# fxxJuses/MICFormer

Hardware: AMD Instinct MI355X
Metric: train volumes/sec (128^3 CT+MRI pair) (higher is better)
Workload: dtype bf16; 1 GPU; MicFormer base Head(embed_dim=48, depths 2-2-6-2, heads 3-6-12-24, window 2^3, 8 classes) full train step (fwd + MDiceLoss + bwd + Adam/cosine) on 128^3 CT+MR pairs, DropPath on; local_batch=2, global_batch=2, parallelism=dp1, launch=hipGraph replay (one graph)

## Files before the change

### micformer_amd/csrc/common.h

```cpp
#pragma once
#include <hip/hip_runtime.h>
#include <stdint.h>

#include "../../include/micformer_hip.h"
#include "gemm_core.h"

#define MICF_RETURN_LAUNCH()                          \
  do {                                                \
    return hipGetLastError() == hipSuccess ? MICF_OK : MICF_ELAUNCH; \
  } while (0)

namespace micf {

struct Options {
  int block_wave = 1;
  int block_recompute_h = 0;
  int block_debug = 0;
  int sample_tile = 1;
  int sample_e = -1;
  int cell_cap = -1;
  int tile_cap_hits = -1, tile_cap_cell = -1, tile_cap_voxel = -1;
};
Options& options();

struct Geo {
  int B, D, H, W;
  FastDiv fW, fH, fD;
  Geo() {}
  Geo(int B_, int D_, int H_, int W_) : B(B_), D(D_), H(H_), W(W_), fW((uint32_t)W_), fH((uint32_t)H_), fD((uint32_t)D_) {}
  __host__ __device__ int64_t tokens() const { return (int64_t)B * D * H * W; }
  __device__ __forceinline__ void decode(int t, int& b, int& d, int& h, int& w) const {
    uint32_t q, r;
    fW.divmod((uint32_t)t, q, r); w = (int)r;
    fH.divmod(q, q, r); h = (int)r;
    fD.divmod(q, q, r); d = (int)r; b = (int)q;
  }
  __device__ __forceinline__ int token(int b, int d, int h, int w) const { return ((b * D + d) * H + h) * W + w; }
};

__device__ __forceinline__ float wave_sum(float v) {
#pragma unroll
  for (int o = 32; o > 0; o >>= 1) v += __shfl_xor(v, o, 64);
  return v;
}

int colsum_atomic(const float* dy, const float* scale, int64_t rps, float* out, int64_t M, int N, hipStream_t s);

constexpr int kOffsetHidden = 16;
struct CellLists {
  int* count;
  int* ovf_count;
  int* list;
  int* ovf;
  int cap;
  float* w8;
};
struct SampleFwdSet { const float *h, *ln_g, *ln_b, *w1, *xa; float *flow, *xs; };
struct SampleBwdSet {
  const float *dxs, *h, *ln_g, *ln_b, *w1, *xa, *flow;
  float *dxa, *dh, *dln_g, *dln_b, *dw1;
  CellLists cl;
  float* partials;
};
int offset_sample_fwd_groups(const SampleFwdSet* sets, int n, int B, int D, int H, int W, int C, float eps, hipStream_t stream);
int offset_sample_bwd_groups(SampleBwdSet* sets, int n, int B, int D, int H, int W, int C, float eps, float* workspace,
                             int64_t workspace_floats, hipStream_t s, int phase = 0);
struct SampleFinishCall { const SampleBwdSet* sets; int n, B, D, H, W, C; float* workspace; int64_t workspace_floats; };
int offset_sample_finish_many(const SampleFinishCall* calls, int ncalls, hipStream_t s);

struct Conv3FwdSet { const float* x1; const float* x2; const float* w; const float* bias; float* y; float* wt; };
struct Conv3BwdSet { const float* dy; const float* w; float* wt; float* dx1; float* dx2; };
int conv3_fwd_x_groups(const Conv3FwdSet* sets, int n, int c1, int c2, int B, int D, int H, int W, int N, hipStream_t stream, int dtype,
                       int prepared, int y_zeroed);
bool conv3_fwd_x_splits(int B, int D, int H, int W, int c1, int c2);
int conv3_bwd_data_x_groups(const Conv3BwdSet* sets, int ng, int c1, int acc1, int c2, int acc2, int B, int D, int H, int W, int N,
                            hipStream_t stream, int dtype, int prepared);

int conv3_bwd_data_x(const float* dy, const float* w, float* wt, float* dx1, int c1, int acc1, float* dx2, int c2, int acc2, int B,
                     int D, int H, int W, int N, hipStream_t stream, int dtype = 0, int prepared = 0);

int64_t conv3_fwdx_workspace(int N, int c1, int c2);
int conv3_fwd_x(const float* x1, int c1, const float* x2, int c2, const float* w, const float* bias, float* y, float* wt, int B, int D,
                int H, int W, int N, hipStream_t stream, int dtype = 0, int prepared = 0);
int64_t conv3_wgradx_workspace(int B, int D, int H, int W, int N, int c1, int c2, int items = 1);
int conv3_wgradx_items(const float* const* dy, const float* const* x1, const float* const* x2, float* const* dw, float* const* dbias,
                       int n, int c1, int c2, int B, int D, int H, int W, int N, float* ws, int64_t ws_floats, hipStream_t stream,
                       int dtype);
int conv3_wgradx(const float* dy, const float* x1, int c1, const float* x2, int c2, float* dw, float* dbias, int B, int D, int H,
                 int W, int N, float* ws, int64_t ws_floats, hipStream_t stream, int dtype = 0);

}
```

### micformer_amd/csrc/linear_grouped.hip

```cpp
#include "common.h"
#include "gemm_dma.h"

namespace micf {

constexpr int kGroupMax = 32;
constexpr int kGroupChunk = 1024;

struct GItem {
  const float* a; const float* dy; const float* scale; float* out; float* dbias; float* dw;
  int M, N, K, rps;
  int tiles_i, tiles, splits, direct;
  int ldw, pad_;
  int64_t split_stride;
};
struct GArgs {
  int n;
  int end[kGroupMax];
  GItem it[kGroupMax];
};

template <bool BF16>
__global__ void __launch_bounds__(256) wgrad_grouped_kernel(const GArgs g) {
  __shared__ __attribute__((aligned(1024))) float Ps[kDmaNS * 64 * kDmaBR];
  __shared__ __attribute__((aligned(1024))) float Qs[kDmaNS * 64 * kDmaBR];
  const int total = g.end[g.n - 1];
  const int w = xcd_order(blockIdx.x, total);
  if (w >= total) return;
  int k = 0;
  while (k < g.n - 1 && w >= g.end[k]) ++k;
  const GItem& it = g.it[k];
  const int local = w - (k ? g.end[k - 1] : 0);
  const int split = local / it.tiles, t = local % it.tiles;
  const int bi = t % it.tiles_i, bj = t / it.tiles_i;
  const int i0 = bi * 64, j0 = bj * 64;
  const int tid = threadIdx.x, lane = tid & 63, wave = __builtin_amdgcn_readfirstlane(tid >> 6);
  const int li = lane & 15, lr = lane >> 4;
  const int r_begin = split * kGroupChunk;
  const int r_end = (r_begin + kGroupChunk < it.M) ? r_begin + kGroupChunk : it.M;
  const DmaOperand P{it.a, it.K, it.K}, Q{it.dy, it.N, it.N};
  const bool do_cs = (it.dbias != nullptr) && (bi == 0) && (tid < 64);

  f32x4 tot[4];
#pragma unroll
  for (int q = 0; q < 4; ++q) tot[q] = f32x4{0.f, 0.f, 0.f, 0.f};
  float ctot = 0.f;
  for (int r = r_begin; r < r_end;) {
    int seg_end = r_end;
    float s = 1.f;
    if (it.scale) {
      const int b = r / it.rps;
      s = it.scale[b];
      const int lim = (b + 1) * it.rps;
      if (lim < seg_end) seg_end = lim;
    }
    f32x4 acc[4];
#pragma unroll
    for (int q = 0; q < 4; ++q) acc[q] = f32x4{0.f, 0.f, 0.f, 0.f};
    float csum = 0.f;
    if (r != r_begin) __syncthreads();
    const int nslab = (seg_end - r) / kDmaBR;
    dma_tile_loop<true, true, kDmaNS, BF16>(P, Q, i0, j0, r, nslab, Ps, Qs, acc, do_cs, csum);
    for (int rr = r + nslab * kDmaBR; rr < seg_end; ++rr) {
      const int jq = j0 + 4 * li + wave;
      float dyv = jq < it.N ? it.dy[(int64_t)rr * it.N + jq] : 0.f;
      if constexpr (BF16) dyv = __uint_as_float(pack_bf16(dyv, 0.f) << 16);
#pragma unroll
      for (int v = 0; v < 4; ++v) {
        const int i = i0 + 16 * lr + 4 * v;
        if (i >= it.K) continue;
        float4 a4 = *reinterpret_cast<const float4*>(it.a + (int64_t)rr * it.K + i);
        if constexpr (BF16) {
          const unsigned lo = pack_bf16(a4.x, a4.y), hi = pack_bf16(a4.z, a4.w);
          a4 = make_float4(__uint_as_float(lo << 16), __uint_as_float(lo & 0xFFFF0000u), __uint_as_float(hi << 16), __uint_as_float(hi & 0xFFFF0000u));
        }
        acc[0][v] += dyv * a4.x; acc[1][v] += dyv * a4.y; acc[2][v] += dyv * a4.z; acc[3][v] += dyv * a4.w;
      }
      if (do_cs && j0 + tid < it.N) csum += it.dy[(int64_t)rr * it.N + j0 + tid];
    }
#pragma unroll
    for (int q = 0; q < 4; ++q) { tot[q][0] += s * acc[q][0]; tot[q][1] += s * acc[q][1]; tot[q][2] += s * acc[q][2]; tot[q][3] += s * acc[q][3]; }
    ctot += s * csum;
    r = seg_end;
  }
  if (do_cs && j0 + tid < it.N) atomicAdd(it.dbias + j0 + tid, ctot);
  const int j = j0 + 4 * li + wave;
  if (j >= it.N) return;
  float* base = it.direct ? it.dw : it.out + (int64_t)split * it.split_stride;
  const int ld = it.direct ? it.ldw : it.K;
#pragma unroll
  for (int v = 0; v < 4; ++v) {
    const int i = i0 + 16 * lr + 4 * v;
    if (i >= it.K) continue;
    float* p = base + (int64_t)j * ld + i;
    float4 o = make_float4(tot[0][v], tot[1][v], tot[2][v], tot[3][v]);
    if (i + 4 <= it.K) {
      if (it.direct) { const float4 old = *reinterpret_cast<const float4*>(p); o.x += old.x; o.y += old.y; o.z += old.z; o.w += old.w; }
      *reinterpret_cast<float4*>(p) = o;
    } else {
      const float e[4] = {o.x, o.y, o.z, o.w};
      for (int q = 0; q < it.K - i; ++q) p[q] = it.direct ? p[q] + e[q] : e[q];
    }
  }
}


constexpr int kB16Piece = 1024 + 64;
constexpr int kB16Stage = 4 * kB16Piece;
typedef short s16x4 __attribute__((ext_vector_type(4)));

__device__ __forceinline__ bf16x8 tr_frag(unsigned stage_piece, int li, int unit0) {
  const int r = li >> 2, u = unit0 + ((li & 3) >> 1);
  const unsigned a0 = stage_piece + (unsigned)((r * 8 + (u ^ (2 * ((r >> 1) & 1)))) * 16 + (li & 1) * 8);
  const unsigned a1 = a0 + 4 * 8 * 16;
  const s16x4 lo = __builtin_amdgcn_ds_read_tr16_b64_v4i16((__attribute__((address_space(3))) s16x4*)(uintptr_t)a0);
  const s16x4 hi = __builtin_amdgcn_ds_read_tr16_b64_v4i16((__attribute__((address_space(3))) s16x4*)(uintptr_t)a1);
  return bf16x8{lo[0], lo[1], lo[2], lo[3], hi[0], hi[1], hi[2], hi[3]};
}

__device__ __forceinline__ void dma16_b16(const uint16_t* gsrc, unsigned lds_byte) {
  dma16(reinterpret_cast<const float*>(gsrc), lds_byte);
}

__global__ void __launch_bounds__(256) wgrad_grouped_b16_kernel(const GArgs g) {
  __shared__ __attribute__((aligned(1024))) char Ps[kDmaNS * kB16Stage];
  __shared__ __attribute__((aligned(1024))) char Qs[kDmaNS * kB16Stage];
  const int total = g.end[g.n - 1];
  const int w = xcd_order(blockIdx.x, total);
  if (w >= total) return;
  int k = 0;
  while (k < g.n - 1 && w >= g.end[k]) ++k;
  const GItem& it = g.it[k];
  const int local = w - (k ? g.end[k - 1] : 0);
  const int split = local / it.tiles, t = local % it.tiles;
  const int bi = t % it.tiles_i, bj = t / it.tiles_i;
  const int i0 = bi * 64, j0 = bj * 64;
  const int tid = threadIdx.x, lane = tid & 63, wave = __builtin_amdgcn_readfirstlane(tid >> 6);
  const int li = lane & 15, lr = lane >> 4;
  const int r_begin = split * kGroupChunk;
  const int r_end = (r_begin + kGroupChunk < it.M) ? r_begin + kGroupChunk : it.M;
  const uint16_t* A = reinterpret_cast<const uint16_t*>(it.a);
  const uint16_t* DY = reinterpret_cast<const uint16_t*>(it.dy);
  const bool do_cs = (it.dbias != nullptr) && (bi == 0);

  const int srow = lane >> 3, sunit = (lane & 7) ^ (2 * ((srow >> 1) & 1));
  int xa = i0 + 8 * sunit; if (xa > it.K - 8) xa = it.K - 8;
  int xd = j0 + 8 * sunit; if (xd > it.N - 8) xd = it.N - 8;
  const unsigned pl = lds_addr(Ps) + wave * kB16Piece, ql = lds_addr(Qs) + wave * kB16Piece;
  const unsigned pf = lds_addr(Ps) + lr * kB16Piece, qf = lds_addr(Qs) + lr * kB16Piece;

  f32x4 tot[4];
#pragma unroll
  for (int q = 0; q < 4; ++q) tot[q] = f32x4{0.f, 0.f, 0.f, 0.f};
  float ctot = 0.f;
  for (int r = r_begin; r < r_end;) {
    int seg_end = r_end;
    float s = 1.f;
    if (it.scale) {
      const int b = r / it.rps;
      s = it.scale[b];
      const int lim = (b + 1) * it.rps;
      if (lim < seg_end) seg_end = lim;
    }
    f32x4 acc[4];
#pragma unroll
    for (int q = 0; q < 4; ++q) acc[q] = f32x4{0.f, 0.f, 0.f, 0.f};
    float csum = 0.f;
    if (r != r_begin) __syncthreads();
    const int nstep = (seg_end - r) / 32;
    const uint16_t* psrc = A + (int64_t)(r + 8 * wave + srow) * it.K + xa;
    const uint16_t* qsrc = DY + (int64_t)(r + 8 * wave + srow) * it.N + xd;
    const int64_t pstep = (int64_t)32 * it.K, qstep = (int64_t)32 * it.N;
#pragma unroll
    for (int st = 0; st < kDmaNS - 1; ++st) {
      if (st < nstep) {
        dma16_b16(psrc, pl + st * kB16Stage);
        dma16_b16(qsrc, ql + st * kB16Stage);
        psrc += pstep; qsrc += qstep;
      }
    }
    for (int st = 0; st < nstep; ++st) {
      wait_younger((nstep - 1 - st < kDmaNS - 2) ? nstep - 1 - st : kDmaNS - 2);
      __builtin_amdgcn_s_barrier();
      if (st + kDmaNS - 1 < nstep) {
        const int buf = (st + kDmaNS - 1) % kDmaNS;
        dma16_b16(psrc, pl + buf * kB16Stage);
        dma16_b16(qsrc, ql + buf * kB16Stage);
        psrc += pstep; qsrc += qstep;
      }
      const unsigned po = pf + (st % kDmaNS) * kB16Stage, qo = qf + (st % kDmaNS) * kB16Stage;
      const bf16x8 bb = tr_frag(qo, li, 2 * wave);
      if (do_cs) {
#pragma unroll
        for (int e = 0; e < 8; ++e) csum += __uint_as_float(((unsigned)(unsigned short)bb[e]) << 16);
      }
#pragma unroll
      for (int q = 0; q < 4; ++q) acc[q] = __builtin_amdgcn_mfma_f32_16x16x32_bf16(tr_frag(po, li, 2 * q), bb, acc[q], 0, 0, 0);
    }
#pragma unroll
    for (int q = 0; q < 4; ++q) { tot[q][0] += s * acc[q][0]; tot[q][1] += s * acc[q][1]; tot[q][2] += s * acc[q][2]; tot[q][3] += s * acc[q][3]; }
    ctot += s * csum;
    r = seg_end;
  }
  const int j = j0 + 16 * wave + li;
  if (do_cs) {
    ctot += __shfl_xor(ctot, 16, 64);
    ctot += __shfl_xor(ctot, 32, 64);
    if (lr == 0 && j < it.N) atomicAdd(it.dbias + j, ctot);
  }
  if (j >= it.N) return;
  float* base = it.direct ? it.dw : it.out + (int64_t)split * it.split_stride;
  const int ld = it.direct ? it.ldw : it.K;
#pragma unroll
  for (int q = 0; q < 4; ++q) {
    const int i = i0 + 16 * q + 4 * lr;
    if (i >= it.K) continue;
    float* p = base + (int64_t)j * ld + i;
    float4 o = make_float4(tot[q][0], tot[q][1], tot[q][2], tot[q][3]);
    if (it.direct) { const float4 old = *reinterpret_cast<const float4*>(p); o.x += old.x; o.y += old.y; o.z += old.z; o.w += old.w; }
    *reinterpret_cast<float4*>(p) = o;
  }
}

__global__ void __launch_bounds__(256) wgrad_grouped_reduce_kernel(const GArgs g) {
  const int w = blockIdx.x;
  int k = 0;
  while (k < g.n - 1 && w >= g.end[k]) ++k;
  const GItem& it = g.it[k];
  const int local = w - (k ? g.end[k - 1] : 0);
  const int64_t n4 = (int64_t)it.N * it.K / 4;
  const int64_t e = (int64_t)local * 256 + threadIdx.x;
  if (e >= n4) return;
  float* dst = it.dw + ((4 * e) / it.K) * (int64_t)it.ldw + (4 * e) % it.K;
  float4 acc = *reinterpret_cast<const float4*>(dst);
  int s = 0;
  for (; s + 4 <= it.splits; s += 4) {
    float4 v[4];
#pragma unroll
    for (int u = 0; u < 4; ++u) v[u] = *reinterpret_cast<const float4*>(it.out + (s + u) * it.split_stride + 4 * e);
#pragma unroll
    for (int u = 0; u < 4; ++u) { acc.x += v[u].x; acc.y += v[u].y; acc.z += v[u].z; acc.w += v[u].w; }
  }
  for (; s < it.splits; ++s) {
    const float4 v = *reinterpret_cast<const float4*>(it.out + s * it.split_stride + 4 * e);
    acc.x += v.x; acc.y += v.y; acc.z += v.z; acc.w += v.w;
  }
  *reinterpret_cast<float4*>(dst) = acc;
}

static bool item_ok(const micf_wgrad_item& x) {
  if (x.operand_dtype != MICF_DTYPE_F32 && x.operand_dtype != MICF_DTYPE_BF16) return false;
  if (x.operand_dtype == MICF_DTYPE_BF16) {
    if (x.M % 32 || x.N % 8 || x.K % 8 || x.N < 8 || x.K < 8) return false;
    if (x.dp_scale && x.rows_per_sample % 32) return false;
  }
  if (!x.a || !x.dy || !x.dw || x.M <= 0 || x.N < 4 || x.K < 4) return false;
  if (x.ldw != 0 && (x.ldw < x.K || x.ldw % 4)) return false;
  if (x.M >= (1LL << 30) || x.N % 4 || x.K % 4) return false;
  if ((reinterpret_cast<uintptr_t>(x.a) | reinterpret_cast<uintptr_t>(x.dy) | reinterpret_cast<uintptr_t>(x.dw)) & 15) return false;
  if (x.dp_scale && (x.rows_per_sample <= 0 || x.M % x.rows_per_sample)) return false;
  return true;
}

static int item_splits(const micf_wgrad_item& x) { return (int)((x.M + kGroupChunk - 1) / kGroupChunk); }

}

using namespace micf;

extern "C" int64_t micf_linear_bwd_weight_grouped_workspace(const micf_wgrad_item* items, int n) {
  if (!items || n <= 0) return 0;
  int64_t total = 0;
  for (int k = 0; k < n; ++k) {
    if (!item_ok(items[k])) return -1;
    const int sp = item_splits(items[k]);
    if (sp > 1) total += (int64_t)sp * items[k].N * items[k].K;
  }
  return total;
}

extern "C" int micf_linear_bwd_weight_grouped(const micf_wgrad_item* items, int n, float* workspace, int64_t workspace_floats,
                                              int dtype, micf_stream_t stream) {
  if (n < 0 || (n > 0 && !items)) return MICF_EINVAL;
  if (n == 0) return MICF_OK;
  const int64_t need = micf_linear_bwd_weight_grouped_workspace(items, n);
  if (need < 0) return MICF_EUNSUPPORTED;
  if (need > 0 && (!workspace || workspace_floats < need || (reinterpret_cast<uintptr_t>(workspace) & 15))) return MICF_EINVAL;
  hipStream_t s = (hipStream_t)stream;
  int64_t ws_off = 0;
  for (int pass = 0; pass < 2; ++pass) {
    int idx[kGroupMax], cnt = 0;
    for (int k = 0; k <= n; ++k) {
      if (k < n && (items[k].operand_dtype == MICF_DTYPE_BF16) == (pass == 1)) idx[cnt++] = k;
      if (cnt == 0 || (cnt < kGroupMax && k < n)) continue;
      GArgs g, rg;
      g.n = cnt;
      rg.n = 0;
      int blocks = 0, rblocks = 0;
      for (int q = 0; q < cnt; ++q) {
        const micf_wgrad_item& x = items[idx[q]];
        GItem& d = g.it[q];
        d.a = x.a; d.dy = x.dy; d.scale = x.dp_scale; d.dbias = x.dbias; d.dw = x.dw;
        d.M = (int)x.M; d.N = x.N; d.K = x.K; d.rps = x.dp_scale ? (int)x.rows_per_sample : (int)x.M;
        d.ldw = x.ldw > 0 ? x.ldw : x.K; d.pad_ = 0;
        d.tiles_i = ceil_div(x.K, 64);
        d.tiles = d.tiles_i * ceil_div(x.N, 64);
        d.splits = item_splits(x);
        d.direct = d.splits == 1;
        d.split_stride = (int64_t)x.N * x.K;
        d.out = d.direct ? nullptr : workspace + ws_off;
        if (!d.direct) ws_off += d.splits * d.split_stride;
        blocks += d.tiles * d.splits;
        g.end[q] = blocks;
        if (!d.direct) {
          rg.it[rg.n] = d;
          rblocks += (int)((d.split_stride / 4 + 255) / 256);
          rg.end[rg.n] = rblocks;
          ++rg.n;
        }
      }
      if (pass == 1) hipLaunchKernelGGL(wgrad_grouped_b16_kernel, dim3((blocks + 7) / 8 * 8), dim3(256), 0, s, g);
      else if (dtype == MICF_DTYPE_BF16) hipLaunchKernelGGL(wgrad_grouped_kernel<true>, dim3((blocks + 7) / 8 * 8), dim3(256), 0, s, g);
      else hipLaunchKernelGGL(wgrad_grouped_kernel<false>, dim3((blocks + 7) / 8 * 8), dim3(256), 0, s, g);
      if (hipGetLastError() != hipSuccess) return MICF_ELAUNCH;
      if (rg.n > 0) {
        hipLaunchKernelGGL(wgrad_grouped_reduce_kernel, dim3(rblocks), dim3(256), 0, s, rg);
        if (hipGetLastError() != hipSuccess) return MICF_ELAUNCH;
      }
      cnt = 0;
    }
  }
  return MICF_OK;
}
```

### micformer_amd/csrc/misc.hip

```cpp
#include <hip/hip_fp16.h>

#include "common.h"
#include <string.h>

namespace micf {

__global__ void __launch_bounds__(256) pad3d_kernel(const float* __restrict__ src, float* __restrict__ dst, int B, int D, int H,
                                                    int W, int Dp, int Hp, int Wp, int C, int64_t total) {
  for (int64_t i = (int64_t)blockIdx.x * 256 + threadIdx.x; i < total; i += (int64_t)gridDim.x * 256) {
    int64_t t = i / C; const int c = (int)(i - t * C);
    const int w = (int)(t % Wp); t /= Wp; const int h = (int)(t % Hp); t /= Hp; const int d = (int)(t % Dp); const int b = (int)(t / Dp);
    dst[i] = (d < D && h < H && w < W) ? src[((((int64_t)b * D + d) * H + h) * W + w) * C + c] : 0.f;
  }
}
__global__ void __launch_bounds__(256) crop3d_kernel(const float* __restrict__ src, float* __restrict__ dst, int B, int D, int H,
                                                     int W, int Dp, int Hp, int Wp, int C, int accumulate, int64_t total) {
  for (int64_t i = (int64_t)blockIdx.x * 256 + threadIdx.x; i < total; i += (int64_t)gridDim.x * 256) {
    int64_t t = i / C; const int c = (int)(i - t * C);
    const int w = (int)(t % W); t /= W; const int h = (int)(t % H); t /= H; const int d = (int)(t % D); const int b = (int)(t / D);
    const float v = src[((((int64_t)b * Dp + d) * Hp + h) * Wp + w) * C + c];
    dst[i] = accumulate ? dst[i] + v : v;
  }
}

__device__ __forceinline__ void ac_coord(int o, int Sin, int Sout, int& i0, int& i1, float& f) {
  const float scale = Sout > 1 ? (float)(Sin - 1) / (float)(Sout - 1) : 0.f;
  const float s = scale * (float)o;
  i0 = (int)s; if (i0 > Sin - 1) i0 = Sin - 1;
  i1 = i0 + (i0 < Sin - 1 ? 1 : 0);
  f = s - (float)i0;
}
template <bool BWD>
__global__ void __launch_bounds__(256) resize_kernel(const float* __restrict__ a, float* __restrict__ o, int B, int D, int H, int W,
                                                     int Do, int Ho, int Wo, int C, int64_t total) {
  for (int64_t i = (int64_t)blockIdx.x * 256 + threadIdx.x; i < total; i += (int64_t)gridDim.x * 256) {
    int64_t t = i / C; const int c = (int)(i - t * C);
    const int w = (int)(t % Wo); t /= Wo; const int h = (int)(t % Ho); t /= Ho; const int d = (int)(t % Do); const int b = (int)(t / Do);
    int d0, d1, h0, h1, w0, w1; float fd, fh, fw;
    ac_coord(d, D, Do, d0, d1, fd); ac_coord(h, H, Ho, h0, h1, fh); ac_coord(w, W, Wo, w0, w1, fw);
    float acc = 0.f;
    const float gv = BWD ? a[i] : 0.f;
#pragma unroll
    for (int q = 0; q < 8; ++q) {
      const int dd = (q & 4) ? d1 : d0, hh = (q & 2) ? h1 : h0, ww = (q & 1) ? w1 : w0;
      const float wt = ((q & 4) ? fd : 1.f - fd) * ((q & 2) ? fh : 1.f - fh) * ((q & 1) ? fw : 1.f - fw);
      const int64_t s = ((((int64_t)b * D + dd) * H + hh) * W + ww) * C + c;
      if (BWD) atomicAdd(o + s, wt * gv); else acc += wt * a[s];
    }
    if (!BWD) o[i] = acc;
  }
}


__global__ void __launch_bounds__(256) sw_window_kernel(const float* __restrict__ vol, float* __restrict__ win, int C, int D, int H,
                                                        int W, int rd, int rh, int rw, int z0, int y0, int x0, int64_t total) {
  for (int64_t i = (int64_t)blockIdx.x * 256 + threadIdx.x; i < total; i += (int64_t)gridDim.x * 256) {
    const int x = (int)(i % rw); int64_t r = i / rw;
    const int y = (int)(r % rh); r /= rh;
    const int z = (int)(r % rd); const int c = (int)(r / rd);
    win[i] = vol[(((int64_t)c * D + z0 + z) * H + y0 + y) * W + x0 + x];
  }
}
__global__ void __launch_bounds__(256) sw_accumulate_kernel(const float* __restrict__ pred, float* __restrict__ out,
                                                            float* __restrict__ count, int K, int D, int H, int W, int rd, int rh,
                                                            int rw, int z0, int y0, int x0, int64_t total) {
  for (int64_t i = (int64_t)blockIdx.x * 256 + threadIdx.x; i < total; i += (int64_t)gridDim.x * 256) {
    const int x = (int)(i % rw); int64_t r = i / rw;
    const int y = (int)(r % rh); r /= rh;
    const int z = (int)(r % rd); const int k = (int)(r / rd);
    const int64_t v = ((int64_t)(z0 + z) * H + y0 + y) * W + x0 + x;
    out[(int64_t)k * D * H * W + v] += pred[i];
    if (k == 0) count[v] += 1.f;
  }
}
__global__ void __launch_bounds__(256) sw_normalize_kernel(float* __restrict__ out, const float* __restrict__ count, int64_t V,
                                                           int64_t total) {
  for (int64_t i = (int64_t)blockIdx.x * 256 + threadIdx.x; i < total; i += (int64_t)gridDim.x * 256) out[i] /= count[i % V];
}

}
using namespace micf;

extern "C" int micf_abi_version(void) { return MICF_ABI_VERSION; }

micf::Options& micf::options() {
  static Options o;
  return o;
}

static int* option_slot(const char* name) {
  if (!name) return nullptr;
  Options& o = micf::options();
  const struct { const char* n; int* v; } table[] = {
      {"block_wave", &o.block_wave}, {"block_recompute_h", &o.block_recompute_h}, {"block_debug", &o.block_debug},
      {"sample_tile", &o.sample_tile}, {"sample_e", &o.sample_e}, {"cell_cap", &o.cell_cap},
      {"tile_cap_hits", &o.tile_cap_hits}, {"tile_cap_cell", &o.tile_cap_cell}, {"tile_cap_voxel", &o.tile_cap_voxel}};
  for (const auto& e : table)
    if (!strcmp(name, e.n)) return e.v;
  return nullptr;
}

extern "C" int micf_set_option(const char* name, int value) {
  int* slot = option_slot(name);
  if (!slot) return MICF_EINVAL;
  *slot = value;
  return MICF_OK;
}

extern "C" int micf_get_option(const char* name, int* value) {
  const int* slot = option_slot(name);
  if (!slot || !value) return MICF_EINVAL;
  *value = *slot;
  return MICF_OK;
}

extern "C" const char* micf_strerror(int code) {
  switch (code) {
    case MICF_OK: return "ok";
    case MICF_EINVAL: return "invalid argument (null pointer, bad size or misaligned buffer)";
    case MICF_EUNSUPPORTED: return "shape not supported by the HIP kernels";
    case MICF_ELAUNCH: return "HIP kernel launch failed";
    default: return "unknown micf error code";
  }
}

static int grid_for(int64_t total) { int64_t b = (total + 255) / 256; return (int)(b > 16384 ? 16384 : (b < 1 ? 1 : b)); }

extern "C" int micf_pad3d(const float* src, float* dst, int B, int D, int H, int W, int Dp, int Hp, int Wp, int C,
                          micf_stream_t stream) {
  if (!src || !dst || B <= 0 || D <= 0 || H <= 0 || W <= 0 || C <= 0 || Dp < D || Hp < H || Wp < W) return MICF_EINVAL;
  const int64_t total = (int64_t)B * Dp * Hp * Wp * C;
  hipLaunchKernelGGL(pad3d_kernel, dim3(grid_for(total)), dim3(256), 0, (hipStream_t)stream, src, dst, B, D, H, W, Dp, Hp, Wp, C, total);
  MICF_RETURN_LAUNCH();
}
extern "C" int micf_crop3d(const float* src, float* dst, int B, int D, int H, int W, int Dp, int Hp, int Wp, int C, int accumulate,
                           micf_stream_t stream) {
  if (!src || !dst || B <= 0 || D <= 0 || H <= 0 || W <= 0 || C <= 0 || Dp < D || Hp < H || Wp < W) return MICF_EINVAL;
  const int64_t total = (int64_t)B * D * H * W * C;
  hipLaunchKernelGGL(crop3d_kernel, dim3(grid_for(total)), dim3(256), 0, (hipStream_t)stream, src, dst, B, D, H, W, Dp, Hp, Wp, C,
                     accumulate, total);
  MICF_RETURN_LAUNCH();
}
extern "C" int micf_resize_trilinear_fwd(const float* src, float* dst, int B, int D, int H, int W, int Do, int Ho, int Wo, int C,
                                         micf_stream_t stream) {
  if (!src || !dst || B <= 0 || D <= 0 || H <= 0 || W <= 0 || Do <= 0 || Ho <= 0 || Wo <= 0 || C <= 0) return MICF_EINVAL;
  const int64_t total = (int64_t)B * Do * Ho * Wo * C;
  hipLaunchKernelGGL(resize_kernel<false>, dim3(grid_for(total)), dim3(256), 0, (hipStream_t)stream, src, dst, B, D, H, W, Do, Ho, Wo, C, total);
  MICF_RETURN_LAUNCH();
}
extern "C" int micf_resize_trilinear_bwd(const float* ddst, float* dsrc, int B, int D, int H, int W, int Do, int Ho, int Wo, int C,
                                         micf_stream_t stream) {
  if (!ddst || !dsrc || B <= 0 || D <= 0 || H <= 0 || W <= 0 || Do <= 0 || Ho <= 0 || Wo <= 0 || C <= 0) return MICF_EINVAL;
  hipStream_t s = (hipStream_t)stream;
  if (hipMemsetAsync(dsrc, 0, sizeof(float) * (size_t)B * D * H * W * C, s) != hipSuccess) return MICF_ELAUNCH;
  const int64_t total = (int64_t)B * Do * Ho * Wo * C;
  hipLaunchKernelGGL(resize_kernel<true>, dim3(grid_for(total)), dim3(256), 0, s, ddst, dsrc, B, D, H, W, Do, Ho, Wo, C, total);
  MICF_RETURN_LAUNCH();
}

extern "C" int micf_sw_window(const float* vol, float* win, int C, int D, int H, int W, int rd, int rh, int rw, int z0, int y0,
                              int x0, micf_stream_t stream) {
  if (!vol || !win || C <= 0 || rd <= 0 || rh <= 0 || rw <= 0 || z0 < 0 || y0 < 0 || x0 < 0 || z0 + rd > D || y0 + rh > H ||
      x0 + rw > W)
    return MICF_EINVAL;
  const int64_t total = (int64_t)C * rd * rh * rw;
  hipLaunchKernelGGL(sw_window_kernel, dim3(grid_for(total)), dim3(256), 0, (hipStream_t)stream, vol, win, C, D, H, W, rd, rh, rw, z0,
                     y0, x0, total);
  MICF_RETURN_LAUNCH();
}
extern "C" int micf_sw_accumulate(const float* pred, float* out, float* count, int K, int D, int H, int W, int rd, int rh, int rw,
                                  int z0, int y0, int x0, micf_stream_t stream) {
  if (!pred || !out || !count || K <= 0 || rd <= 0 || rh <= 0 || rw <= 0 || z0 < 0 || y0 < 0 || x0 < 0 || z0 + rd > D ||
      y0 + rh > H || x0 + rw > W)
    return MICF_EINVAL;
  const int64_t total = (int64_t)K * rd * rh * rw;
  hipLaunchKernelGGL(sw_accumulate_kernel, dim3(grid_for(total)), dim3(256), 0, (hipStream_t)stream, pred, out, count, K, D, H, W, rd,
                     rh, rw, z0, y0, x0, total);
  MICF_RETURN_LAUNCH();
}
extern "C" int micf_sw_normalize(float* out, const float* count, int K, int64_t V, micf_stream_t stream) {
  if (!out || !count || K <= 0 || V <= 0) return MICF_EINVAL;
  const int64_t total = (int64_t)K * V;
  hipLaunchKernelGGL(sw_normalize_kernel, dim3(grid_for(total)), dim3(256), 0, (hipStream_t)stream, out, count, V, total);
  MICF_RETURN_LAUNCH();
}

extern "C" int micf_zero(void* p, int64_t bytes, micf_stream_t stream) {
  if (!p || bytes < 0) return MICF_EINVAL;
  if (bytes == 0) return MICF_OK;
  return hipMemsetAsync(p, 0, (size_t)bytes, (hipStream_t)stream) == hipSuccess ? MICF_OK : MICF_ELAUNCH;
}

namespace micf {
__device__ __forceinline__ uint64_t mix64(uint64_t z) {
  z += 0x9E3779B97F4A7C15ull;
  z = (z ^ (z >> 30)) * 0xBF58476D1CE4E5B9ull;
  z = (z ^ (z >> 27)) * 0x94D049BB133111EBull;
  return z ^ (z >> 31);
}
__global__ void __launch_bounds__(256) drop_path_draw_kernel(uint64_t* __restrict__ rng, const float* __restrict__ keep,
                                                             float* __restrict__ out, int n, int B) {
  const uint64_t seed = rng[0], ctr = rng[1];
  for (int e = threadIdx.x; e < n * B; e += 256) {
    const float k = keep[e / B];
    const uint64_t h = mix64(mix64(seed ^ mix64(ctr)) + (uint64_t)e);
    const float u = (float)(h >> 40) * (1.0f / 16777216.0f);
    out[e] = (u < k) ? 1.0f / k : 0.0f;
  }
  __syncthreads();
  if (threadIdx.x == 0) rng[1] = ctr + 1;
}
}

extern "C" int micf_drop_path_draw(void* rng, const float* keep, float* out, int n, int B, micf_stream_t stream) {
  if (!rng || !keep || !out || n < 0 || B <= 0) return MICF_EINVAL;
  if (n == 0) return MICF_OK;
  hipLaunchKernelGGL(micf::drop_path_draw_kernel, dim3(1), dim3(256), 0, (hipStream_t)stream, static_cast<uint64_t*>(rng), keep, out, n, B);
  MICF_RETURN_LAUNCH();
}

namespace micf {
constexpr int kPrepMax = 64;
struct PrepArgs {
  int n;
  int end[kPrepMax];
  const float* src[kPrepMax]; void* dst[kPrepMax]; void* dst_t[kPrepMax];
  int rows[kPrepMax], cols[kPrepMax], bf16[kPrepMax];
};
__device__ __forceinline__ unsigned pack_bf16(float a, float b) {
  typedef __bf16 bf16x2_hw __attribute__((ext_vector_type(2)));
  typedef float f32x2_hw __attribute__((ext_vector_type(2)));
  const f32x2_hw f = {a, b};
  return __builtin_bit_cast(unsigned, __builtin_convertvector(f, bf16x2_hw));
}
__device__ __forceinline__ void prep_store4(void* base, int64_t idx, bool bf16, bool vec, int valid, float4 v) {
  if (bf16) {
    uint16_t* d = static_cast<uint16_t*>(base) + idx;
    if (vec) { *reinterpret_cast<uint2*>(d) = make_uint2(pack_bf16(v.x, v.y), pack_bf16(v.z, v.w)); return; }
    const float e[4] = {v.x, v.y, v.z, v.w};
    for (int i = 0; i < valid; ++i) d[i] = (uint16_t)(pack_bf16(e[i], 0.f) & 0xFFFFu);
  } else {
    float* d = static_cast<float*>(base) + idx;
    if (vec) { *reinterpret_cast<float4*>(d) = v; return; }
    const float e[4] = {v.x, v.y, v.z, v.w};
    for (int i = 0; i < valid; ++i) d[i] = e[i];
  }
}
__global__ void __launch_bounds__(256) weight_prep_kernel(const PrepArgs a) {
  __shared__ float t[64][65];
  const int w = blockIdx.x;
  int k = 0;
  while (k < a.n - 1 && w >= a.end[k]) ++k;
  const int local = w - (k ? a.end[k - 1] : 0);
  const int rows = a.rows[k], cols = a.cols[k];
  const bool bf = a.bf16[k] == 1 || a.bf16[k] == 2, blocked = a.bf16[k] >= 2;
  auto at = [&](int r, int c, int Cn) {
    return blocked ? ((int64_t)(r >> 4) * (Cn >> 4) + (c >> 4)) * 256 + (r & 15) * 16 + (c & 15) : (int64_t)r * Cn + c;
  };
  const int tc = (cols + 63) >> 6;
  const int r0 = (local / tc) * 64, c0 = (local % tc) * 64;
  const int tx = threadIdx.x & 15, ty = threadIdx.x >> 4;
  const float* __restrict__ src = a.src[k];
  const bool vc = (cols & 3) == 0, vr = (rows & 3) == 0;
#pragma unroll
  for (int j = 0; j < 64; j += 16) {
    const int r = r0 + ty + j, c = c0 + 4 * tx;
    float4 v = make_float4(0.f, 0.f, 0.f, 0.f);
    const int valid = r < rows ? (cols - c < 4 ? cols - c : 4) : 0;
    if (valid == 4 && vc) v = *reinterpret_cast<const float4*>(src + (int64_t)r * cols + c);
    else if (valid > 0) {
      float e[4] = {0.f, 0.f, 0.f, 0.f};
      for (int i = 0; i < valid; ++i) e[i] = src[(int64_t)r * cols + c + i];
      v = make_float4(e[0], e[1], e[2], e[3]);
    }
    if (a.dst[k] && valid > 0) prep_store4(a.dst[k], at(r, c, cols), bf, valid == 4 && vc, valid, v);
    t[ty + j][4 * tx] = v.x; t[ty + j][4 * tx + 1] = v.y; t[ty + j][4 * tx + 2] = v.z; t[ty + j][4 * tx + 3] = v.w;
  }
  if (!a.dst_t[k]) return;
  __syncthreads();
#pragma unroll
  for (int j = 0; j < 64; j += 16) {
    const int c = c0 + ty + j, r = r0 + 4 * tx;
    const int valid = c < cols ? (rows - r < 4 ? rows - r : 4) : 0;
    if (valid <= 0) continue;
    const float4 v = make_float4(t[4 * tx][ty + j], t[4 * tx + 1][ty + j], t[4 * tx + 2][ty + j], t[4 * tx + 3][ty + j]);
    prep_store4(a.dst_t[k], at(c, r, rows), bf, valid == 4 && vr, valid, v);
  }
}
}

extern "C" int micf_weight_prep_grouped(const micf_weight_prep_item* items, int n, micf_stream_t stream) {
  if (n < 0 || (n > 0 && !items)) return MICF_EINVAL;
  for (int first = 0; first < n; first += micf::kPrepMax) {
    const int cnt = (n - first < micf::kPrepMax) ? n - first : micf::kPrepMax;
    micf::PrepArgs a;
    a.n = cnt;
    int blocks = 0;
    for (int k = 0; k < cnt; ++k) {
      const micf_weight_prep_item& it = items[first + k];
      const int align = (it.bf16 == 1 || it.bf16 == 2) ? 7 : 15;
      if (it.bf16 < 0 || it.bf16 > 3 || (it.bf16 >= 2 && ((it.rows | it.cols) & 15))) return MICF_EINVAL;
      if (!it.src || (!it.dst && !it.dst_t) || it.rows <= 0 || it.cols <= 0 || (reinterpret_cast<uintptr_t>(it.src) & 15) ||
          (reinterpret_cast<uintptr_t>(it.dst) & align) || (reinterpret_cast<uintptr_t>(it.dst_t) & align))
        return MICF_EINVAL;
      a.src[k] = it.src; a.dst[k] = it.dst; a.dst_t[k] = it.dst_t; a.rows[k] = it.rows; a.cols[k] = it.cols; a.bf16[k] = it.bf16;
      blocks += ((it.rows + 63) / 64) * ((it.cols + 63) / 64);
      a.end[k] = blocks;
    }
    hipLaunchKernelGGL(micf::weight_prep_kernel, dim3(blocks), dim3(256), 0, (hipStream_t)stream, a);
    if (hipGetLastError() != hipSuccess) return MICF_ELAUNCH;
  }
  return MICF_OK;
}

namespace micf {
constexpr int kSwMax = 64;
struct SwCoords { int n; int b[kSwMax], z[kSwMax], y[kSwMax], x[kSwMax]; };
__global__ void __launch_bounds__(256) sw_window_batch_kernel(const float* __restrict__ vol, float* __restrict__ win, SwCoords c, int C,
                                                              int D, int H, int W, int rd, int rh, int rw, int64_t per) {
  const int n = blockIdx.y;
  const float* v = vol + (int64_t)c.b[n] * C * D * H * W;
  float* o = win + (int64_t)n * per;
  for (int64_t i = (int64_t)blockIdx.x * 256 + threadIdx.x; i < per; i += (int64_t)gridDim.x * 256) {
    const int x = (int)(i % rw); int64_t r = i / rw;
    const int y = (int)(r % rh); r /= rh;
    const int z = (int)(r % rd); const int ch = (int)(r / rd);
    o[i] = v[(((int64_t)ch * D + c.z[n] + z) * H + c.y[n] + y) * W + c.x[n] + x];
  }
}
__global__ void __launch_bounds__(256) sw_accumulate_batch_kernel(const float* __restrict__ pred, float* __restrict__ out,
                                                                  float* __restrict__ count, SwCoords c, int K, int D, int H, int W,
                                                                  int rd, int rh, int rw, int64_t per) {
  const int n = blockIdx.y;
  const float* p = pred + (int64_t)n * per;
  float* o = out + (int64_t)c.b[n] * K * D * H * W;
  float* cn = count + (int64_t)c.b[n] * D * H * W;
  for (int64_t i = (int64_t)blockIdx.x * 256 + threadIdx.x; i < per; i += (int64_t)gridDim.x * 256) {
    const int x = (int)(i % rw); int64_t r = i / rw;
    const int y = (int)(r % rh); r /= rh;
    const int z = (int)(r % rd); const int k = (int)(r / rd);
    const int64_t v = ((int64_t)(c.z[n] + z) * H + c.y[n] + y) * W + c.x[n] + x;
    atomicAdd(o + (int64_t)k * D * H * W + v, p[i]);
    if (k == 0) atomicAdd(cn + v, 1.f);
  }
}
static bool sw_coords(SwCoords& c, const int32_t* coords, int n, int B, int D, int H, int W, int rd, int rh, int rw) {
  if (!coords || n <= 0 || n > kSwMax) return false;
  c.n = n;
  for (int i = 0; i < n; ++i) {
    c.b[i] = coords[4 * i]; c.z[i] = coords[4 * i + 1]; c.y[i] = coords[4 * i + 2]; c.x[i] = coords[4 * i + 3];
    if (c.b[i] < 0 || c.b[i] >= B || c.z[i] < 0 || c.y[i] < 0 || c.x[i] < 0 || c.z[i] + rd > D || c.y[i] + rh > H || c.x[i] + rw > W) return false;
  }
  return true;
}
}

extern "C" int micf_sw_window_batch(const float* vol, float* win, const int32_t* coords, int n, int B, int C, int D, int H, int W,
                                    int rd, int rh, int rw, micf_stream_t stream) {
  micf::SwCoords c;
  if (!vol || !win || C <= 0 || rd <= 0 || rh <= 0 || rw <= 0 || !micf::sw_coords(c, coords, n, B, D, H, W, rd, rh, rw)) return MICF_EINVAL;
  const int64_t per = (int64_t)C * rd * rh * rw;
  hipLaunchKernelGGL(micf::sw_window_batch_kernel, dim3(grid_for(per) > 2048 ? 2048 : grid_for(per), n), dim3(256), 0, (hipStream_t)stream,
                     vol, win, c, C, D, H, W, rd, rh, rw, per);
  MICF_RETURN_LAUNCH();
}
extern "C" int micf_sw_accumulate_batch(const float* pred, float* out, float* count, const int32_t* coords, int n, int B, int K, int D,
                                        int H, int W, int rd, int rh, int rw, micf_stream_t stream) {
  micf::SwCoords c;
  if (!pred || !out || !count || K <= 0 || rd <= 0 || rh <= 0 || rw <= 0 || !micf::sw_coords(c, coords, n, B, D, H, W, rd, rh, rw))
    return MICF_EINVAL;
  const int64_t per = (int64_t)K * rd * rh * rw;
  hipLaunchKernelGGL(micf::sw_accumulate_batch_kernel, dim3(grid_for(per) > 2048 ? 2048 : grid_for(per), n), dim3(256), 0,
                     (hipStream_t)stream, pred, out, count, c, K, D, H, W, rd, rh, rw, per);
  MICF_RETURN_LAUNCH();
}

namespace micf {
template <class T> __device__ __forceinline__ float ldv(const T* p, int64_t i);
template <> __device__ __forceinline__ float ldv<float>(const float* p, int64_t i) { return p[i]; }
template <> __device__ __forceinline__ float ldv<__half>(const __half* p, int64_t i) { return __half2float(p[i]); }

template <class T>
__global__ void __launch_bounds__(256) intensity_stats_kernel(const T* __restrict__ vol, double* __restrict__ sums, int64_t V, int chunks) {
  const int plane = blockIdx.y;
  const int64_t per = (V + chunks - 1) / chunks;
  const int64_t v0 = blockIdx.x * per, v1 = (v0 + per < V) ? v0 + per : V;
  const T* p = vol + (int64_t)plane * V;
  float a = 0.f, b = 0.f, c = 0.f;
  for (int64_t i = v0 + threadIdx.x; i < v1; i += 256) {
    const float x = ldv<T>(p, i);
    if (x != 0.f) { a += x; b += x * x; c += 1.f; }
  }
  a = wave_sum(a); b = wave_sum(b); c = wave_sum(c);
  __shared__ float part[4][3];
  const int wave = threadIdx.x >> 6;
  if ((threadIdx.x & 63) == 0) { part[wave][0] = a; part[wave][1] = b; part[wave][2] = c; }
  __syncthreads();
  if (threadIdx.x < 3) {
    const int q = threadIdx.x;
    atomicAdd(sums + plane * 3 + q, (double)part[0][q] + (double)part[1][q] + (double)part[2][q] + (double)part[3][q]);
  }
}
template <class T>
__global__ void __launch_bounds__(256) input_prepare_kernel(const T* __restrict__ vol, const double* __restrict__ sums,
                                                            const float* __restrict__ params, float* __restrict__ out,
                                                            const uint8_t* __restrict__ lab_in, uint8_t* __restrict__ lab_out, int Cm, int D,
                                                            int H, int W) {
  const int b = blockIdx.y;
  const int64_t V = (int64_t)D * H * W;
  int fd = 0, fh = 0, fw = 0;
  float f = 0.f, o = 0.f;
  if (params) { fd = params[b * 5] != 0.f; fh = params[b * 5 + 1] != 0.f; fw = params[b * 5 + 2] != 0.f; f = params[b * 5 + 3]; o = params[b * 5 + 4]; }
  for (int64_t i = (int64_t)blockIdx.x * 256 + threadIdx.x; i < V; i += (int64_t)gridDim.x * 256) {
    const int w = (int)(i % W); int64_t r = i / W;
    const int h = (int)(r % H); const int d = (int)(r / H);
    const int64_t src = ((int64_t)(fd ? D - 1 - d : d) * H + (fh ? H - 1 - h : h)) * W + (fw ? W - 1 - w : w);
    for (int m = 0; m < (out ? Cm : 0); ++m) {
      const double* sp = sums + ((int64_t)b * Cm + m) * 3;
      const double n = sp[2];
      const double mean = n > 0 ? sp[0] / n : 0.0;
      double var = n > 0 ? sp[1] / n - mean * mean : 0.0;
      if (var < 0) var = 0;
      double sd = sqrt(var);
      if (sd == 0.0) sd = 1.0;
      const float x = ldv<T>(vol, ((int64_t)b * Cm + m) * V + src);
      float y = x != 0.f ? (float)(((double)x - mean) / sd) : 0.f;
      out[((int64_t)b * Cm + m) * V + i] = y * (1.f + f) + o;
    }
    if (lab_in) lab_out[(int64_t)b * V + i] = lab_in[(int64_t)b * V + src];
  }
}
template <class T>
__global__ void __launch_bounds__(256) patch_rows_prepared_kernel(const T* __restrict__ vol, const double* __restrict__ sums,
                                                                  const float* __restrict__ params, float* __restrict__ rows0,
                                                                  float* __restrict__ rows1, int B, int Cm, int D, int H, int W, int k,
                                                                  int Dc, int Hc, int Wc, int64_t total4) {
  const int m = blockIdx.y;
  float* rows = m == 0 ? rows0 : rows1;
  const int64_t i = (int64_t)blockIdx.x * 256 + threadIdx.x;
  if (i >= total4 || !rows) return;
  const int K3 = k * k * k, q4 = K3 >> 2;
  const int t4 = (int)(i % q4);
  int64_t r = i / q4;
  const int xc = (int)(r % Wc); int64_t r2 = r / Wc;
  const int yc = (int)(r2 % Hc); r2 /= Hc;
  const int zc = (int)(r2 % Dc); const int b = (int)(r2 / Dc);
  int fd = 0, fh = 0, fw = 0;
  float f = 0.f, o = 0.f;
  if (params) { fd = params[b * 5] != 0.f; fh = params[b * 5 + 1] != 0.f; fw = params[b * 5 + 2] != 0.f; f = params[b * 5 + 3]; o = params[b * 5 + 4]; }
  const double* sp = sums + ((int64_t)b * Cm + m) * 3;
  const double n = sp[2];
  const double mean = n > 0 ? sp[0] / n : 0.0;
  double var = n > 0 ? sp[1] / n - mean * mean : 0.0;
  if (var < 0) var = 0;
  double sd = sqrt(var);
  if (sd == 0.0) sd = 1.0;
  const int64_t V = (int64_t)D * H * W;
  float v[4] = {0.f, 0.f, 0.f, 0.f};
#pragma unroll
  for (int j = 0; j < 4; ++j) {
    const int tap = 4 * t4 + j;
    const int tz = tap / (k * k), ty = (tap / k) % k, tx = tap % k;
    const int z = zc * k + tz, y = yc * k + ty, x = xc * k + tx;
    if (z >= D || y >= H || x >= W) continue;
    const int64_t src = ((int64_t)(fd ? D - 1 - z : z) * H + (fh ? H - 1 - y : y)) * W + (fw ? W - 1 - x : x);
    const float raw = ldv<T>(vol, ((int64_t)b * Cm + m) * V + src);
    const float yv = raw != 0.f ? (float)(((double)raw - mean) / sd) : 0.f;
    v[j] = yv * (1.f + f) + o;
  }
  *reinterpret_cast<float4*>(rows + r * K3 + 4 * t4) = make_float4(v[0], v[1], v[2], v[3]);
}
}

extern "C" int micf_patch_rows_prepared(const void* vol, int is_half, const double* sums, const float* params, float* rows0,
                                        float* rows1, int B, int Cm, int D, int H, int W, int k, micf_stream_t stream) {
  if (!vol || !sums || (!rows0 && !rows1) || B <= 0 || Cm < 1 || Cm > 2 || (Cm == 1 && rows1) || D <= 0 || H <= 0 || W <= 0 ||
      (k != 2 && k != 4))
    return MICF_EINVAL;
  if ((reinterpret_cast<uintptr_t>(rows0) | reinterpret_cast<uintptr_t>(rows1)) & 15) return MICF_EINVAL;
  const int Dc = (D + k - 1) / k, Hc = (H + k - 1) / k, Wc = (W + k - 1) / k;
  const int64_t total4 = (int64_t)B * Dc * Hc * Wc * (k * k * k / 4);
  const dim3 grid((unsigned)((total4 + 255) / 256), Cm);
  if (is_half) hipLaunchKernelGGL(micf::patch_rows_prepared_kernel<__half>, grid, dim3(256), 0, (hipStream_t)stream, static_cast<const __half*>(vol), sums, params, rows0, rows1, B, Cm, D, H, W, k, Dc, Hc, Wc, total4);
  else hipLaunchKernelGGL(micf::patch_rows_prepared_kernel<float>, grid, dim3(256), 0, (hipStream_t)stream, static_cast<const float*>(vol), sums, params, rows0, rows1, B, Cm, D, H, W, k, Dc, Hc, Wc, total4);
  MICF_RETURN_LAUNCH();
}

extern "C" int micf_intensity_stats(const void* vol, int is_half, double* sums, int B, int Cm, int64_t V, micf_stream_t stream) {
  if (!vol || !sums || B <= 0 || Cm <= 0 || V <= 0) return MICF_EINVAL;
  hipStream_t s = (hipStream_t)stream;
  if (hipMemsetAsync(sums, 0, sizeof(double) * 3 * B * Cm, s) != hipSuccess) return MICF_ELAUNCH;
  int chunks = (int)((V + 65535) / 65536);
  if (chunks > 256) chunks = 256;
  if (is_half) hipLaunchKernelGGL(micf::intensity_stats_kernel<__half>, dim3(chunks, B * Cm), dim3(256), 0, s, static_cast<const __half*>(vol), sums, V, chunks);
  else hipLaunchKernelGGL(micf::intensity_stats_kernel<float>, dim3(chunks, B * Cm), dim3(256), 0, s, static_cast<const float*>(vol), sums, V, chunks);
  MICF_RETURN_LAUNCH();
}
extern "C" int micf_input_prepare(const void* vol, int is_half, const double* sums, const float* params, float* out,
                                  const uint8_t* label_in, uint8_t* label_out, int B, int Cm, int D, int H, int W, micf_stream_t stream) {
  if (!vol || !sums || (!out && !label_in) || B <= 0 || Cm <= 0 || D <= 0 || H <= 0 || W <= 0 || (label_in && !label_out)) return MICF_EINVAL;
  const int64_t V = (int64_t)D * H * W;
  const dim3 grid(grid_for(V) > 1024 ? 1024 : grid_for(V), B);
  if (is_half) hipLaunchKernelGGL(micf::input_prepare_kernel<__half>, grid, dim3(256), 0, (hipStream_t)stream, static_cast<const __half*>(vol), sums, params, out, label_in, label_out, Cm, D, H, W);
  else hipLaunchKernelGGL(micf::input_prepare_kernel<float>, grid, dim3(256), 0, (hipStream_t)stream, static_cast<const float*>(vol), sums, params, out, label_in, label_out, Cm, D, H, W);
  MICF_RETURN_LAUNCH();
}
```

Measured before the change: 237.7 pairs/s.

## Add full-width bf16 wgrad kernel covering whole N×K per block with adaptive row chunks

Adds a specialised bf16 weight-gradient kernel for the transformer's common channel shapes (48/96/192/384). Each block computes the entire N×K output tile over a row chunk, using a 4-stage LDS ring with DMA loads, transposed LDS reads and MFMA. The row chunk shrinks adaptively so there are enough blocks. This removes the 64×64 tile decomposition and its re-reading of the activations and dy, and it fuses the dbias column sum into the kernel. The cost is more split partials going through the reduce kernel, plus higher LDS and register pressure per block.

```diff
diff --git a/micformer_amd/csrc/common.h b/micformer_amd/csrc/common.h
--- a/micformer_amd/csrc/common.h
+++ b/micformer_amd/csrc/common.h
@@ -20,6 +20,7 @@
   int sample_e = -1;
   int cell_cap = -1;
   int tile_cap_hits = -1, tile_cap_cell = -1, tile_cap_voxel = -1;
+  int wgrad_fullwidth = 1;
 };
 Options& options();
 
diff --git a/micformer_amd/csrc/linear_grouped.hip b/micformer_amd/csrc/linear_grouped.hip
--- a/micformer_amd/csrc/linear_grouped.hip
+++ b/micformer_amd/csrc/linear_grouped.hip
@@ -10,7 +10,8 @@
   const float* a; const float* dy; const float* scale; float* out; float* dbias; float* dw;
   int M, N, K, rps;
   int tiles_i, tiles, splits, direct;
-  int ldw, pad_;
+  int ldw, chunk;
+  int cps, pad_;
   int64_t split_stride;
 };
 struct GArgs {
@@ -221,6 +222,175 @@
   }
 }
 
+constexpr int kFwNS = 4;
+
+template <int W>
+struct FwImage {
+  static_assert(W == 48 || W == 96 || W == 192 || W == 384, "operand width");
+  static constexpr int U = W / 8;
+  static constexpr int S = 2 * W;
+  static constexpr int kPad = W == 48 ? 128 : (W == 96 ? 32 : (W == 192 ? 64 : 128));
+  static constexpr int kPiece = 8 * S + kPad;
+  static constexpr int kStage = 4 * kPiece;
+  static constexpr int kDma = (8 * U + 63) / 64;
+  __device__ static __forceinline__ int swz(int row) { return W == 192 ? 2 * ((row >> 1) & 1) : (W == 384 ? 2 * (row & 3) : 0); }
+  __device__ static __forceinline__ int src(int wave, int lane, int i) {
+    const int s = 64 * i + lane;
+    if (s >= 8 * U) return -1;
+    const int row = s / U, su = s - row * U;
+    return (8 * wave + row) * S + 16 * (su ^ swz(row));
+  }
+  __device__ static __forceinline__ bf16x8 frag(unsigned lane_base, unsigned swl, int t) {
+    const unsigned a0 = lane_base + ((unsigned)(32 * t) ^ swl);
+    const unsigned a1 = a0 + 4 * S;
+    const s16x4 lo = __builtin_amdgcn_ds_read_tr16_b64_v4i16((__attribute__((address_space(3))) s16x4*)(uintptr_t)a0);
+    const s16x4 hi = __builtin_amdgcn_ds_read_tr16_b64_v4i16((__attribute__((address_space(3))) s16x4*)(uintptr_t)a1);
+    return bf16x8{lo[0], lo[1], lo[2], lo[3], hi[0], hi[1], hi[2], hi[3]};
+  }
+};
+
+template <int N>
+__device__ __forceinline__ void wait_vmcnt() { asm volatile("s_waitcnt vmcnt(%0)" ::"n"(N) : "memory"); }
+template <int D>
+__device__ __forceinline__ void wait_younger_stages(int younger) {
+  static_assert(2 * D < 64, "vmcnt range");
+  if (younger <= 0) wait_vmcnt<0>();
+  else if (younger == 1) wait_vmcnt<D>();
+  else wait_vmcnt<2 * D>();
+}
+
+template <int KT, int NT>
+constexpr int fw_stage_bytes() { return FwImage<16 * KT>::kStage + FwImage<16 * NT>::kStage; }
+constexpr int kFwLds32 = kFwNS * fw_stage_bytes<3, 12>();
+constexpr int kFwLds16 = kFwNS * fw_stage_bytes<6, 24>();
+
+template <int KT, int NT>
+__device__ __forceinline__ void wgrad_fullwidth_unit(const GItem& it, int split, char* ring) {
+  using PA = FwImage<16 * KT>;
+  using PB = FwImage<16 * NT>;
+  constexpr int WK = (NT % 4 == 0) ? 1 : ((KT % 4 == 0) ? 4 : ((KT % 2 == 0 && NT % 2 == 0) ? 2 : 1));
+  constexpr int WN = 4 / WK;
+  constexpr int IA = (KT + WK - 1) / WK, JB = (NT + WN - 1) / WN;
+  constexpr int D = PA::kDma + PB::kDma;
+  constexpr int kStage = PA::kStage + PB::kStage;
+  static_assert(kFwNS == 4, "wait_younger_stages covers a ring of four");
+  const int tid = threadIdx.x, lane = tid & 63, wave = __builtin_amdgcn_readfirstlane(tid >> 6);
+  const int li = lane & 15, lr = lane >> 4;
+  const int wk = wave % WK, wn = wave / WK;
+  const int seg = split / it.cps, c = split - seg * it.cps;
+  const int r_begin = seg * it.rps + c * it.chunk;
+  const int r_end = (c + 1) * it.chunk < it.rps ? r_begin + it.chunk : (seg + 1) * it.rps;
+  const int nstep = (r_end - r_begin) / 32;
+  const bool do_cs = (it.dbias != nullptr) && (wk == 0);
+
+  int pa_off[PA::kDma], pb_off[PB::kDma];
+#pragma unroll
+  for (int i = 0; i < PA::kDma; ++i) pa_off[i] = PA::src(wave, lane, i);
+#pragma unroll
+  for (int i = 0; i < PB::kDma; ++i) pb_off[i] = PB::src(wave, lane, i);
+  const char* pa = reinterpret_cast<const char*>(it.a) + (int64_t)r_begin * PA::S;
+  const char* pb = reinterpret_cast<const char*>(it.dy) + (int64_t)r_begin * PB::S;
+  const unsigned ring0 = lds_addr(ring);
+  const unsigned la = ring0 + wave * PA::kPiece, lb = ring0 + PA::kStage + wave * PB::kPiece;
+  auto issue = [&](int buf) {
+    const unsigned da = __builtin_amdgcn_readfirstlane(la + buf * kStage), db = __builtin_amdgcn_readfirstlane(lb + buf * kStage);
+#pragma unroll
+    for (int i = 0; i < PA::kDma; ++i)
+      if (64 * (i + 1) <= 8 * PA::U || pa_off[i] >= 0) dma16_b16(reinterpret_cast<const uint16_t*>(pa + pa_off[i]), da + i * 1024);
+#pragma unroll
+    for (int i = 0; i < PB::kDma; ++i)
+      if (64 * (i + 1) <= 8 * PB::U || pb_off[i] >= 0) dma16_b16(reinterpret_cast<const uint16_t*>(pb + pb_off[i]), db + i * 1024);
+    pa += 32 * PA::S; pb += 32 * PB::S;
+  };
+  const int r4 = li >> 2;
+  const unsigned fa = ring0 + lr * PA::kPiece + r4 * PA::S + (li & 3) * 8;
+  const unsigned fb = ring0 + PA::kStage + lr * PB::kPiece + r4 * PB::S + (li & 3) * 8;
+  const unsigned swa = 16 * PA::swz(r4), swb = 16 * PB::swz(r4);
+
+  f32x4 acc[IA][JB];
+  float csum[JB];
+#pragma unroll
+  for (int b = 0; b < JB; ++b) {
+    csum[b] = 0.f;
+#pragma unroll
+    for (int a = 0; a < IA; ++a) acc[a][b] = f32x4{0.f, 0.f, 0.f, 0.f};
+  }
+#pragma unroll
+  for (int st = 0; st < kFwNS - 1; ++st)
+    if (st < nstep) issue(st);
+  for (int st = 0; st < nstep; ++st) {
+    wait_younger_stages<D>((nstep - 1 - st < kFwNS - 2) ? nstep - 1 - st : kFwNS - 2);
+    __builtin_amdgcn_s_barrier();
+    if (st + kFwNS - 1 < nstep) issue((st + kFwNS - 1) % kFwNS);
+    const unsigned so = (st % kFwNS) * kStage;
+    bf16x8 bb[JB];
+#pragma unroll
+    for (int b = 0; b < JB; ++b) {
+      const int jt = wn + WN * b;
+      if (NT % WN == 0 || jt < NT) {
+        bb[b] = PB::frag(fb + so, swb, jt);
+        if (do_cs) {
+#pragma unroll
+          for (int e = 0; e < 8; ++e) csum[b] += __uint_as_float(((unsigned)(unsigned short)bb[b][e]) << 16);
+        }
+      }
+    }
+#pragma unroll
+    for (int a = 0; a < IA; ++a) {
+      const int kt = wk + WK * a;
+      if (KT % WK == 0 || kt < KT) {
+        const bf16x8 aa = PA::frag(fa + so, swa, kt);
+#pragma unroll
+        for (int b = 0; b < JB; ++b)
+          if (NT % WN == 0 || wn + WN * b < NT) acc[a][b] = __builtin_amdgcn_mfma_f32_16x16x32_bf16(aa, bb[b], acc[a][b], 0, 0, 0);
+      }
+    }
+  }
+  const float s = it.scale ? it.scale[seg] : 1.f;
+  float* base = it.out + (int64_t)split * it.split_stride;
+#pragma unroll
+  for (int b = 0; b < JB; ++b) {
+    const int jt = wn + WN * b;
+    if (NT % WN != 0 && jt >= NT) continue;
+    const int j = 16 * jt + li;
+    if (do_cs) {
+      float cs = s * csum[b];
+      cs += __shfl_xor(cs, 16, 64);
+      cs += __shfl_xor(cs, 32, 64);
+      if (lr == 0) atomicAdd(it.dbias + j, cs);
+    }
+#pragma unroll
+    for (int a = 0; a < IA; ++a) {
+      const int kt = wk + WK * a;
+      if (KT % WK != 0 && kt >= KT) continue;
+      float* p = base + (int64_t)j * it.K + 16 * kt + 4 * lr;
+      *reinterpret_cast<float4*>(p) = make_float4(s * acc[a][b][0], s * acc[a][b][1], s * acc[a][b][2], s * acc[a][b][3]);
+    }
+  }
+}
+
+template <int CLS>
+__global__ void __launch_bounds__(256) wgrad_fullwidth_b16_kernel(const GArgs g) {
+  __shared__ __attribute__((aligned(1024))) char ring[CLS == 0 ? kFwLds32 : kFwLds16];
+  const int w = blockIdx.x;
+  int k = 0;
+  while (k < g.n - 1 && w >= g.end[k]) ++k;
+  const GItem& it = g.it[k];
+  const int split = w - (k ? g.end[k - 1] : 0);
+  const int kt = it.K >> 4, nt = it.N >> 4;
+  if constexpr (CLS == 0) {
+    if (kt == 12) wgrad_fullwidth_unit<12, 3>(it, split, ring);
+    else if (nt == 3) wgrad_fullwidth_unit<3, 3>(it, split, ring);
+    else if (nt == 6) wgrad_fullwidth_unit<3, 6>(it, split, ring);
+    else wgrad_fullwidth_unit<3, 12>(it, split, ring);
+  } else {
+    if (kt == 24) wgrad_fullwidth_unit<24, 6>(it, split, ring);
+    else if (nt == 6) wgrad_fullwidth_unit<6, 6>(it, split, ring);
+    else if (nt == 12) wgrad_fullwidth_unit<6, 12>(it, split, ring);
+    else wgrad_fullwidth_unit<6, 24>(it, split, ring);
+  }
+}
+
 __global__ void __launch_bounds__(256) wgrad_grouped_reduce_kernel(const GArgs g) {
   const int w = blockIdx.x;
   int k = 0;
@@ -261,7 +431,34 @@
   return true;
 }
 
-static int item_splits(const micf_wgrad_item& x) { return (int)((x.M + kGroupChunk - 1) / kGroupChunk); }
+static int fw_class(const micf_wgrad_item& x) {
+  if (options().wgrad_fullwidth == 0 || x.operand_dtype != MICF_DTYPE_BF16 || x.M <= kGroupChunk) return -1;
+  if ((x.K == 48 && (x.N == 48 || x.N == 96 || x.N == 192)) || (x.K == 192 && x.N == 48)) return 0;
+  if ((x.K == 96 && (x.N == 96 || x.N == 192 || x.N == 384)) || (x.K == 384 && x.N == 96)) return 1;
+  return -1;
+}
+
+static int fw_chunk(const micf_wgrad_item& x) {
+  const int forced = options().wgrad_fullwidth;
+  if (forced >= 32) return (forced > kGroupChunk ? kGroupChunk : forced) / 32 * 32;
+  int c = kGroupChunk;
+  while (c > 256 && x.M / c < 128) c >>= 1;
+  return c;
+}
+static int fw_cps(const micf_wgrad_item& x) {
+  const int64_t rps = x.dp_scale ? x.rows_per_sample : x.M;
+  const int c = fw_chunk(x);
+  return (int)((rps + c - 1) / c);
+}
+
+static int item_splits(const micf_wgrad_item& x) {
+  if (fw_class(x) >= 0) return (int)(x.M / (x.dp_scale ? x.rows_per_sample : x.M)) * fw_cps(x);
+  return (int)((x.M + kGroupChunk - 1) / kGroupChunk);
+}
+static int item_kernel(const micf_wgrad_item& x) {
+  const int cls = fw_class(x);
+  return cls >= 0 ? 2 + cls : (x.operand_dtype == MICF_DTYPE_BF16 ? 1 : 0);
+}
 
 }
 
@@ -287,10 +484,10 @@
   if (need > 0 && (!workspace || workspace_floats < need || (reinterpret_cast<uintptr_t>(workspace) & 15))) return MICF_EINVAL;
   hipStream_t s = (hipStream_t)stream;
   int64_t ws_off = 0;
-  for (int pass = 0; pass < 2; ++pass) {
+  for (int pass = 0; pass < 4; ++pass) {
     int idx[kGroupMax], cnt = 0;
     for (int k = 0; k <= n; ++k) {
-      if (k < n && (items[k].operand_dtype == MICF_DTYPE_BF16) == (pass == 1)) idx[cnt++] = k;
+      if (k < n && item_kernel(items[k]) == pass) idx[cnt++] = k;
       if (cnt == 0 || (cnt < kGroupMax && k < n)) continue;
       GArgs g, rg;
       g.n = cnt;
@@ -302,8 +499,10 @@
         d.a = x.a; d.dy = x.dy; d.scale = x.dp_scale; d.dbias = x.dbias; d.dw = x.dw;
         d.M = (int)x.M; d.N = x.N; d.K = x.K; d.rps = x.dp_scale ? (int)x.rows_per_sample : (int)x.M;
         d.ldw = x.ldw > 0 ? x.ldw : x.K; d.pad_ = 0;
-        d.tiles_i = ceil_div(x.K, 64);
-        d.tiles = d.tiles_i * ceil_div(x.N, 64);
+        d.tiles_i = pass >= 2 ? 1 : ceil_div(x.K, 64);
+        d.tiles = pass >= 2 ? 1 : d.tiles_i * ceil_div(x.N, 64);
+        d.chunk = pass >= 2 ? fw_chunk(x) : kGroupChunk;
+        d.cps = pass >= 2 ? fw_cps(x) : 0;
         d.splits = item_splits(x);
         d.direct = d.splits == 1;
         d.split_stride = (int64_t)x.N * x.K;
@@ -318,7 +517,9 @@
           ++rg.n;
         }
       }
-      if (pass == 1) hipLaunchKernelGGL(wgrad_grouped_b16_kernel, dim3((blocks + 7) / 8 * 8), dim3(256), 0, s, g);
+      if (pass == 2) hipLaunchKernelGGL(wgrad_fullwidth_b16_kernel<0>, dim3(blocks), dim3(256), 0, s, g);
+      else if (pass == 3) hipLaunchKernelGGL(wgrad_fullwidth_b16_kernel<1>, dim3(blocks), dim3(256), 0, s, g);
+      else if (pass == 1) hipLaunchKernelGGL(wgrad_grouped_b16_kernel, dim3((blocks + 7) / 8 * 8), dim3(256), 0, s, g);
       else if (dtype == MICF_DTYPE_BF16) hipLaunchKernelGGL(wgrad_grouped_kernel<true>, dim3((blocks + 7) / 8 * 8), dim3(256), 0, s, g);
       else hipLaunchKernelGGL(wgrad_grouped_kernel<false>, dim3((blocks + 7) / 8 * 8), dim3(256), 0, s, g);
       if (hipGetLastError() != hipSuccess) return MICF_ELAUNCH;
diff --git a/micformer_amd/csrc/misc.hip b/micformer_amd/csrc/misc.hip
--- a/micformer_amd/csrc/misc.hip
+++ b/micformer_amd/csrc/misc.hip
@@ -94,7 +94,8 @@
   const struct { const char* n; int* v; } table[] = {
       {"block_wave", &o.block_wave}, {"block_recompute_h", &o.block_recompute_h}, {"block_debug", &o.block_debug},
       {"sample_tile", &o.sample_tile}, {"sample_e", &o.sample_e}, {"cell_cap", &o.cell_cap},
-      {"tile_cap_hits", &o.tile_cap_hits}, {"tile_cap_cell", &o.tile_cap_cell}, {"tile_cap_voxel", &o.tile_cap_voxel}};
+      {"tile_cap_hits", &o.tile_cap_hits}, {"tile_cap_cell", &o.tile_cap_cell}, {"tile_cap_voxel", &o.tile_cap_voxel},
+      {"wgrad_fullwidth", &o.wgrad_fullwidth}};
   for (const auto& e : table)
     if (!strcmp(name, e.n)) return e.v;
   return nullptr;
```

New measurement: 232.7 pairs/s. 0.979x the previous value.
